# thecasterian/fluca

Hardware: AMD Instinct MI355X
Metric: pressure-Poisson Jacobi-PCG iterations/s, 512^3 cells per GPU (higher is better)
Workload: dtype f64

## Files before the change

fluca_amd/csrc/fl_cheb2.hip:

```cpp
#include <type_traits>

#include "fl_device.h"
#include "fl_handle.h"

namespace fl {

typedef double v2d_t __attribute__((ext_vector_type(2)));
template <int NT>
__device__ __forceinline__ double2 c2_ld2(const double *p)
{
  if (NT) {
    const v2d_t v = __builtin_nontemporal_load(reinterpret_cast<const v2d_t *>(p));
    return make_double2(v.x, v.y);
  }
  return *reinterpret_cast<const double2 *>(p);
}
template <int NT>
__device__ __forceinline__ void c2_st2(double *p, double2 v)
{
  if (NT) {
    v2d_t t;
    t.x = v.x;
    t.y = v.y;
    __builtin_nontemporal_store(t, reinterpret_cast<v2d_t *>(p));
  } else *reinterpret_cast<double2 *>(p) = v;
}

template <int NT>
__device__ __forceinline__ double2 c2_LD2(const double *base, unsigned byteoff) { return c2_ld2<NT>(reinterpret_cast<const double *>(reinterpret_cast<const char *>(base) + byteoff)); }
__device__ __forceinline__ double c2_LD1(const double *base, unsigned byteoff) { return *reinterpret_cast<const double *>(reinterpret_cast<const char *>(base) + byteoff); }
template <int NT>
__device__ __forceinline__ void c2_ST2(double *base, unsigned byteoff, double2 v) { c2_st2<NT>(reinterpret_cast<double *>(reinterpret_cast<char *>(base) + byteoff), v); }
__device__ __forceinline__ void c2_ST1(double *base, unsigned byteoff, double v) { *reinterpret_cast<double *>(reinterpret_cast<char *>(base) + byteoff) = v; }

__device__ __forceinline__ int c2_wrap(int gi, int n, int per, bool &in)
{
  if (gi < 0) {
    const int m = per & 3;
    in = m != 0;
    return m == 1 ? gi + n : (m == 2 ? gi : 0);
  }
  if (gi >= n) {
    const int m = (per >> 2) & 3;
    in = m != 0;
    return m == 1 ? gi - n : (m == 2 ? gi : n - 1);
  }
  in = true;
  return gi;
}

__device__ __forceinline__ int c2_xcd_remap(int b, int nblocks) { return (nblocks & 7) ? b : (b & 7) * (nblocks >> 3) + (b >> 3); }

template <int RY, int NW, bool JAC, int NT, bool MGD = false, int Z = 0>
__global__ void __launch_bounds__(64 * NW) k_cheb2(GridP g, int perx, int pery, int perz, const double *X0, const double *X1, double *X0w, double *X1w, const double *__restrict__ b, const double *D0, const double *D1, double *D0w,
                                                  double *D1w, const KspScal *__restrict__ s, double *__restrict__ partial, int stride, int zc, int tiles_x, int tiles, int remap, const double *__restrict__ zq = nullptr,
                                                  const double *__restrict__ za_dev = nullptr, double *__restrict__ bw = nullptr)
{
  constexpr bool ZR = Z != 0, ZS = Z == 2;
  static_assert(!(ZR && MGD), "the three-step sweep is the pre-smoother: no sums of the outer iteration");
  constexpr int TX = 128, TY = NW * RY, LX = TX + 4, NTH = 64 * NW;
  constexpr int NTL = NT >= 2, NTS = NT >= 1;
  __shared__ __attribute__((aligned(16))) double XJ[3][TY + 4][LX];
  __shared__ __attribute__((aligned(16))) double XN[3][TY + 2][LX];
  __shared__ double                              red[6 * NW], cB[2 * TY][5];
  if (s->reason != 0) return;

  const double *x  = s->cur ? X1 : X0;
  double       *xn = s->cur ? X0w : X1w;
  const double *d  = s->dcur ? D1 : D0;
  double       *dn = s->dcur ? D0w : D1w;
  double        rho0 = s->cheb_rho, c0 = s->cheb_c;
  double        rho1, c1;
  const double  cf = s->cheb_c;
  const double  za = ZS ? *za_dev : 0.;
  {
    double ck, ckm1;
    cheb_advance(s, s->ck, s->ckm1, ck, ckm1, rho1, c1);
    if (ZR) {
      rho0 = rho1;
      c0   = c1;
      double ck2, ckm2;
      cheb_advance(s, ck, ckm1, ck2, ckm2, rho1, c1);
    }
  }

  const int bb    = remap ? c2_xcd_remap(blockIdx.x, gridDim.x) : blockIdx.x;
  const int chunk = bb / tiles, tile = bb % tiles;
  const int i0 = (tile % tiles_x) * TX, j0 = (tile / tiles_x) * TY;
  const int k0 = chunk * zc, k1 = min(k0 + zc, g.nz);
  const int tid = threadIdx.x, lane = tid & 63;
  const int w   = __builtin_amdgcn_readfirstlane(tid >> 6);
  const int ie = min(TX, g.nx - i0), je = min(TY, g.ny - j0);
// ... 253 lines not shown
        const double2 below = *reinterpret_cast<const double2 *>(&XJ[bp][rlr][lc]);
        const double  west = XJ[bc][rlr][lc - 1], east = XJ[bc][rlr][lc + 2];
        const double  dyz = Ayc + z1c;
        const double  v0 = (xc0 + dyz) * cen.x + xl0 * west + xh0 * cen.y + Ayl * south.x + Ayh * north.x + z1l * below.x + z1h * C.hxR.x;
        const double  v1 = (xc1 + dyz) * cen.y + xl1 * cen.x + xh1 * east + Ayl * south.y + Ayh * north.y + z1l * below.y + z1h * C.hxR.y;
        const double2 bm = ZR ? zb1R : C.hbR, dm = ZR ? cen : C.hdR;
        const double  r0 = bm.x - v0, r1 = bm.y - v1;
        const double  z0 = JAC ? r0 / (xc0 + dyz) : r0, z1 = JAC ? r1 / (xc1 + dyz) : r1;
        const double  e0 = (rho0 != 0. ? rho0 * dm.x : 0.) + c0 * z0;
        const double  e1 = (rho0 != 0. ? rho0 * dm.y : 0.) + c0 * z1;
        hx1R.x = (rinn0 && pin1) ? cen.x + e0 : 0.;
        hx1R.y = (rinn1 && pin1) ? cen.y + e1 : 0.;
      }
      if (anyB) {
        const double cen = XJ[bc][HB.lr][HB.lc], dyz = cB[tbc][4] + z1c;
        const double v = dyz * cen + cB[tbc][0] * XJ[bc][HB.lr][HB.lc - 1] + cB[tbc][1] * XJ[bc][HB.lr][HB.lc + 1] + cB[tbc][2] * XJ[bc][HB.lr - 1][HB.lc] + cB[tbc][3] * XJ[bc][HB.lr + 1][HB.lc] + z1l * XJ[bp][HB.lr][HB.lc] + z1h * C.hxB;
        const double r = (ZR ? zb1B : C.hbB) - v, z = JAC ? r / dyz : r;
        const double e = (rho0 != 0. ? rho0 * (ZR ? cen : C.hdB) : 0.) + c0 * z;
        hx1B = (HB.in && pin1) ? cen + e : 0.;
      }
    }

    if constexpr (DO2) {
      const int     bc = (k2 + 3) % 3, bp = (k2 + 2) % 3;
      const int64_t p2 = (int64_t)k2 * g.sxy;
#pragma unroll
      for (int m = 0; m < RY; ++m) {
        const int     lr    = w * RY + m + 1;
        const double2 cen   = *reinterpret_cast<const double2 *>(&XN[bc][lr][lc]);
        const double2 south = *reinterpret_cast<const double2 *>(&XN[bc][lr - 1][lc]);
        const double2 north = *reinterpret_cast<const double2 *>(&XN[bc][lr + 1][lc]);
        const double2 below = *reinterpret_cast<const double2 *>(&XN[bp][lr][lc]);
        const double  west = XN[bc][lr][lc - 1], east = XN[bc][lr][lc + 2];
        const double  dyz = yc[m] + z2c;
        const double  v0 = (xc0 + dyz) * cen.x + xl0 * west + xh0 * cen.y + yl[m] * south.x + yh[m] * north.x + z2l * below.x + z2h * x1v[m].x;
        const double  v1 = (xc1 + dyz) * cen.y + xl1 * cen.x + xh1 * east + yl[m] * south.y + yh[m] * north.y + z2l * below.y + z2h * x1v[m].y;
        const double  r0 = sb2[m].x - v0, r1 = sb2[m].y - v1;
        const double  z0 = JAC ? r0 / (xc0 + dyz) : r0, z1 = JAC ? r1 / (xc1 + dyz) : r1;
        double2       e, xo;
        e.x  = rho1 * d1p[m].x + c1 * z0;
        e.y  = rho1 * d1p[m].y + c1 * z1;
        xo.x = cen.x + e.x;
        xo.y = cen.y + e.y;
        if (rin[m] && in0) {
          if (in1) {
            c2_ST2<NTS>(dn + rob[m] + p2, lo, e);
            c2_ST2<NTS>(xn + rob[m] + p2, lo, xo);
            if (MGD) {
              acc[0] += xo.x + xo.y;
              acc[1] += xo.x * xo.x + xo.y * xo.y;
              acc[2] += sb2[m].x * xo.x + sb2[m].y * xo.y;
              acc[3] += sb2[m].x + sb2[m].y;
              acc[4] += sb2[m].x * sb2[m].x + sb2[m].y * sb2[m].y;
            } else {
              acc[3] += z0 + z1;
              acc[4] += z0 * z0 + z1 * z1;
              acc[5] += r0 * r0 + r1 * r1;
            }
          } else {
            c2_ST1(dn + rob[m] + p2, lo, e.x);
            c2_ST1(xn + rob[m] + p2, lo, xo.x);
            if (MGD) {
              acc[0] += xo.x;
              acc[1] += xo.x * xo.x;
              acc[2] += sb2[m].x * xo.x;
              acc[3] += sb2[m].x;
              acc[4] += sb2[m].x * sb2[m].x;
            } else {
              acc[3] += z0;
              acc[4] += z0 * z0;
              acc[5] += r0 * r0;
            }
          }
        }
      }
    }

    {
      const int bj = (kk + 3) % 3, bn = (kc + 3) % 3;
#pragma unroll
      for (int m = 0; m < RY; ++m) {
        if (rin[m]) {
          if (in1) {
            *reinterpret_cast<double2 *>(&XJ[bj][w * RY + m + 2][lc]) = C.x[m];
            if constexpr (DO1) *reinterpret_cast<double2 *>(&XN[bn][w * RY + m + 1][lc]) = x1v[m];
          } else if (in0) {
            XJ[bj][w * RY + m + 2][lc] = C.x[m].x;
            if constexpr (DO1) XN[bn][w * RY + m + 1][lc] = x1v[m].x;
          }
        }
      }
      if (rok1) {
        *reinterpret_cast<double2 *>(&XJ[bj][rlr][lc]) = C.hxR;
        if constexpr (DO1)
          if (rowA) *reinterpret_cast<double2 *>(&XN[bn][rlr - 1][lc]) = hx1R;
      } else if (rok0) {
        XJ[bj][rlr][lc] = C.hxR.x;
        if constexpr (DO1)
          if (rowA) XN[bn][rlr - 1][lc] = hx1R.x;
      }
// ... 73 lines not shown
}

int fl_cheb2_agree(fl_poisson *h)
{
  if (h->cheb2_agreed[0] >= 0) return 0;
  const bool legal = fl_cheb2_usable(h);
  double     no[2] = {legal ? 0. : 1., (legal && h->ncell >= 32768) ? 0. : 1.};
  if (h->multi) {
    FL_CHK(fl_allreduce_sum(h, &no[0]));
    FL_CHK(fl_allreduce_sum(h, &no[1]));
  }
  h->cheb2_agreed[0] = no[0] == 0. ? 1 : 0;
  h->cheb2_agreed[1] = no[1] == 0. ? 1 : 0;
  return 0;
}

Cheb2Plan fl_cheb2_plan(const GridP &g)
{
  Cheb2Plan p;
  p.nw      = g.ny > 8 ? 8 : 4;
  p.tiles_x = (g.nx + 127) / 128;
  const int ty    = 2 * p.nw;
  const int tiles = p.tiles_x * ((g.ny + ty - 1) / ty);
  p.tiles         = tiles;
  int nchunk = z_chunk_count(tiles, g.nz, 256, 16);
  if (tiles * nchunk > 256 && tiles <= 256) nchunk = std::max(1, 256 / tiles);
  const ZChunks z = z_chunks(g.nz, nchunk);
  p.zc      = z.zc;
  p.nchunk  = z.nchunk;
  p.nblocks = tiles * p.nchunk;
  return p;
}

template <int NW, bool JAC, bool MGD = false, int Z = 0>
static void cheb2_t(fl_poisson *h, const Cheb2Plan &p, double *X0, double *X1, const double *B, double *D0, double *D1, const double *zq = nullptr, const double *za_dev = nullptr, double *bw = nullptr)
{
  int per[3];
  for (int d = 0; d < 3; ++d) {
    int m[2];
    for (int side = 0; side < 2; ++side) m[side] = (h->multi && h->nbr[2 * d + side] >= 0 && !h->wrap_local[d]) ? 2 : (h->ax[d].periodic ? 1 : 0);
    per[d] = m[0] | (m[1] << 2);
  }
  hipLaunchKernelGGL((k_cheb2<2, NW, JAC, 2, MGD, Z>), dim3(p.nblocks), dim3(64 * NW), 0, h->stream, h->g, per[0], per[1], per[2], X0, X1, X0, X1, B, D0, D1, D0, D1, h->scal, h->partial, h->partial_stride, p.zc, p.tiles_x, p.tiles, 1,
                     zq, za_dev, bw);
}

void fl_launch_cheb2_from_zero(fl_poisson *h, const Cheb2Plan &p, bool jac, double *X0, double *X1, const double *B, double *D0, double *D1, const double *subq, const double *suba_dev, double *Bw)
{
  if (subq) {
    if (p.nw == 8) {
      if (jac) cheb2_t<8, true, false, 2>(h, p, X0, X1, B, D0, D1, subq, suba_dev, Bw);
      else cheb2_t<8, false, false, 2>(h, p, X0, X1, B, D0, D1, subq, suba_dev, Bw);
    } else {
      if (jac) cheb2_t<4, true, false, 2>(h, p, X0, X1, B, D0, D1, subq, suba_dev, Bw);
      else cheb2_t<4, false, false, 2>(h, p, X0, X1, B, D0, D1, subq, suba_dev, Bw);
    }
    return;
  }
  if (p.nw == 8) {
    if (jac) cheb2_t<8, true, false, 1>(h, p, X0, X1, B, D0, D1);
    else cheb2_t<8, false, false, 1>(h, p, X0, X1, B, D0, D1);
  } else {
    if (jac) cheb2_t<4, true, false, 1>(h, p, X0, X1, B, D0, D1);
    else cheb2_t<4, false, false, 1>(h, p, X0, X1, B, D0, D1);
  }
}

void fl_launch_cheb2(fl_poisson *h, const Cheb2Plan &p, bool jac, double *X0, double *X1, const double *B, double *D0, double *D1, bool mgdots)
{
  if (mgdots) {
    if (p.nw == 8) cheb2_t<8, true, true>(h, p, X0, X1, B, D0, D1);
    else cheb2_t<4, true, true>(h, p, X0, X1, B, D0, D1);
    return;
  }
  if (p.nw == 8) {
    if (jac) cheb2_t<8, true>(h, p, X0, X1, B, D0, D1);
    else cheb2_t<8, false>(h, p, X0, X1, B, D0, D1);
  } else {
    if (jac) cheb2_t<4, true>(h, p, X0, X1, B, D0, D1);
    else cheb2_t<4, false>(h, p, X0, X1, B, D0, D1);
  }
}
```

fluca_amd/csrc/fl_handle.h:

```cpp
#pragma once
#include <algorithm>
#include <cmath>
#include <cstdlib>
#include <cstring>
#include <limits>
#include <list>
#include <string>

#include "fl_internal.h"
#include "fl_knobs.h"

typedef struct ncclComm *ncclComm_t;

namespace fl {

void launch_pad_copy(hipStream_t, const GridP &, const double *, double *);
void launch_unpad_copy(hipStream_t, const GridP &, const double *, double *, const double *);
void launch_project_all(hipStream_t, const GridP &, const double *p, double *const v[3], double *const V[3]);
bool project_six_usable(const GridP &, const double *p_unpadded, double *const v[3], double *const V[3]);
void launch_project_six(hipStream_t, const GridP &, const double *p, bool direct, int per, double *const v[3], double *const V[3]);
void launch_wrap(hipStream_t, const GridP &, double *, int axis, int nvec = 1, int64_t vstride = 0);
void launch_pack_faces_sr(hipStream_t, const GridP &, const double *r, const double *sb, const double *W, const KspScal *s, double *const bufs[6]);
void launch_face_ext(hipStream_t, const GridP &, double *v, double *buf, int axis, int side, int ea, int eb, int mode);
void launch_face_ext_deep(hipStream_t, const GridP &, double *v, double *buf, int axis, int side, int ea, int eb, int dp, int mode);
// ... 188 lines not shown
    *count_out = cnt;
  }
  ~ProfEvents()
  {
    for (hipEvent_t e : ev) (void)hipEventDestroy(e);
  }
};

inline int fl_plane_size(const fl_poisson *h, int d) { return d == 0 ? h->g.ny * h->g.nz : (d == 1 ? h->g.nx * h->g.nz : h->g.nx * h->g.ny); }
int  fl_dev_alloc(fl_poisson *h, void **p, size_t bytes, bool zero);
int  fl_ensure_vec(fl_poisson *h, double **v);
void fl_vmm_destroy(fl_poisson *h);
int  fl_ensure_partials(fl_poisson *h, int nblocks);
int  fl_ensure_hist(fl_poisson *h, int nhist);
int  fl_zero_vec(fl_poisson *h, double *v);
int  fl_halo_messages(const fl_poisson *h, bool self, fl_halo_msg plan[12]);
int  fl_fill_ghosts(fl_poisson *h, double *v);
int  fl_fill_ghosts_full(fl_poisson *h, double *v);
int  fl_fill_ghosts_deep(fl_poisson *h, double *v);
int  fl_fill_hifaces(fl_poisson *h, const double *const V[3]);
int  fl_exchange_r_begin(fl_poisson *h, double *r, const double *q);
int  fl_exchange_sr_begin(fl_poisson *h, const double *r, const double *sb, const double *W, double *rn);
int  fl_exchange_r_end(fl_poisson *h, double *r);
bool fl_any_ghost_exchange(const fl_poisson *h);
int fl_allreduce_max(fl_poisson *h, double *v);
int fl_allreduce_sum(fl_poisson *h, double *v);
int fl_poll_scal(fl_poisson *h);
int fl_apply_tiled(fl_poisson *h, const double *xpad, double *y, int unpadded_y);
int fl_residual(fl_poisson *h, const double *x, const double *b, double *r);
int fl_residual_padded(fl_poisson *h, double *xpad, const double *bpad, double *rpad);
bool fl_residual_restrict_fusable(const GridP &g);
int fl_residual_restrict_padded(fl_poisson *h, double *xpad, const double *bpad, const double *wx, const double *wy, const double *wz, fl_poisson *hc, double *cpad);
int fl_apply_padded_dot(fl_poisson *h, double *xpad, double *ypad, double *xy);
int fl_cheb_smooth_padded(fl_poisson *h, int nu, bool jac, bool guess_zero, bool *mgdots = nullptr, const double *subq = nullptr, const double *suba_dev = nullptr);
int fl_solve_cg(fl_poisson *h, const double *b, double *x, const fl_ksp_opts *o, fl_ksp_stats *st);
int fl_solve_bcgs(fl_poisson *h, const double *b, double *x, const fl_ksp_opts *o, fl_ksp_stats *st);
int fl_solve_cg_sr(fl_poisson *h, const double *b, double *x, const fl_ksp_opts *o, fl_ksp_stats *st);
int fl_ksp_begin(fl_poisson *h, const fl_ksp_opts *o);
int fl_bcgs_fin_step(fl_poisson *h, int mode, int nblocks, int nslot, int nhist);
int fl_ksp_finish(fl_poisson *h, const fl_ksp_opts *o, fl_ksp_stats *st);
int fl_cheb_begin(fl_poisson *h, const fl_ksp_opts *o, double emin, double emax);
int fl_cheb_fin_step(fl_poisson *h, int nblocks, int nhist);
int fl_solve_cheb(fl_poisson *h, const double *b, double *x, const fl_ksp_opts *o, fl_ksp_stats *st);
double fl_gershgorin_bound(const fl_poisson *h, bool jac);
struct Cheb2Plan {
  int nw, tiles_x, tiles, nchunk, zc, nblocks;
};
bool      fl_cheb2_usable(const fl_poisson *h);
int       fl_cheb2_agree(fl_poisson *h);
Cheb2Plan fl_cheb2_plan(const GridP &g);
void      fl_launch_cheb2(fl_poisson *h, const Cheb2Plan &p, bool jac, double *X0, double *X1, const double *B, double *D0, double *D1, bool mgdots = false);
namespace fl {
struct SchurVarT {
  const double *w0[3], *w1[3];
  const int    *c0[3];
};
}
bool      fl_schur_var_usable(const fl_poisson *h);
int       fl_schur_var_fill_ghosts(fl_poisson *h, double *p_pad);
int       fl_schur_var_apply_fused(fl_poisson *h, const fl::SchurVarT &t, const double *ainv, const double *p_pad, double *y);
struct SchurVarPlan {
  int     per_xcd, nseg, band, fixed_seg;
  int64_t items;
};
SchurVarPlan schur_var_plan(const fl::GridP &g);
struct TP {
  int ry, nchunk, zc, tiles_x, nblocks;
};
TP tile_plan(const fl::GridP &g);
void      fl_launch_cheb2_from_zero(fl_poisson *h, const Cheb2Plan &p, bool jac, double *X0, double *X1, const double *B, double *D0, double *D1, const double *subq, const double *suba_dev, double *Bw);
int  fl_solve_cg_mg(fl_poisson *h, const double *b, double *x, const fl_ksp_opts *o, fl_ksp_stats *st);
void fl_mg_destroy(fl_poisson *h);
void fl_mg_set_stream(fl_poisson *h);
```

fluca_amd/csrc/fl_knobs.h:

```cpp
#pragma once
#include <atomic>

#define FL_PUBLIC_KNOBS(X)                                                                                                                   \
  X(cheb_fuse, 1)                   \
  X(placement, 0)                           \
  X(cg_xbatch, 1)                                           \
  X(cg_xdepth, 8)                 \
  X(cheb_zero3, 1)                  \
  X(mg_prolong, 1)                                                             \
  X(mg_flexible, 1)                                                             \
  X(mg_coarse, 1)                                   \
  X(mg_post_smooth, 0)               \
  X(schur_var_fused, 1)      \
  X(overlap, 1)              \
  X(comm_loopback, 0)           \
  X(comm_trace, 0)                             \
  X(ghost_width, 0)                                       \
  X(placement_verbose, 0)                                                                        \
  X(placement_vmm, 1)                    \
  X(allreduce, 0)

namespace fl {

enum Knob : int {
#define X(n, d) K_##n,
  FL_PUBLIC_KNOBS(X)
#undef X
      K_COUNT
};

int         knob(Knob k);
void        knob_set(Knob k, int v);
int         knob_find(const char *name);
const char *knob_name(int k);

}
```

fluca_amd/csrc/fl_ksp.hip:

```cpp
#include <ctime>
#include "fl_handle.h"
#include "fl_device.h"
#include "fl_stencil.h"

namespace fl {

__device__ __forceinline__ double2 LD2(const double *base, unsigned byteoff) { return *reinterpret_cast<const double2 *>(reinterpret_cast<const char *>(base) + byteoff); }
__device__ __forceinline__ void    ST2(double *base, unsigned byteoff, double2 v) { *reinterpret_cast<double2 *>(reinterpret_cast<char *>(base) + byteoff) = v; }
__device__ __forceinline__ void    ST1(double *base, unsigned byteoff, double v) { *reinterpret_cast<double *>(reinterpret_cast<char *>(base) + byteoff) = v; }
__device__ __forceinline__ double uniform(double v)
{
  const int lo = __builtin_amdgcn_readfirstlane(__double2loint(v)), hi = __builtin_amdgcn_readfirstlane(__double2hiint(v));
  return __hiloint2double(hi, lo);
}


struct Tile {
  int  i, il, k0, k1, lane, w, j0w, i0;
  bool own0, own1;
};
template <int RY>
__device__ __forceinline__ Tile make_tile(const GridP &g, int nchunk, int zc, int tiles_x)
{
  Tile      t;
// ... 1045 lines not shown
  return !((g.nx & 1) || (g.ny & 1) || (g.nz & 1));
}

int fl_residual_restrict_padded(fl_poisson *h, double *xpad, const double *bpad, const double *wx, const double *wy, const double *wz, fl_poisson *hc, double *cpad)
{
  const GridP &g = h->g, &gc = hc->g;
  if (!fl_residual_restrict_fusable(g)) return 1;
  if (gc.nx * 2 != g.nx || gc.ny * 2 != g.ny || gc.nz * 2 != g.nz) return 1;
  const PlanA p = plan_cg_A(g, 0, 0);
  FL_CHK(fl_fill_ghosts(h, xpad));
  StAux ax;
  ax.csx  = gc.sx;
  ax.csxy = gc.sxy;
  ax.coff = gc.off0;
  if (p.nw == 8) bcgs_st_t<2, 8, 11>(h, p, false, xpad, bpad, wx, wy, cpad, const_cast<double *>(wz), ax);
  else bcgs_st_t<2, 4, 11>(h, p, false, xpad, bpad, wx, wy, cpad, const_cast<double *>(wz), ax);
  return 0;
}

int fl_apply_padded_dot(fl_poisson *h, double *xpad, double *ypad, double *xy)
{
  FL_CHK(fl_fill_ghosts(h, xpad));
  const PlanA pa = plan_cg_A(h->g, 0, 0);
  FL_CHK(fl_ensure_partials(h, pa.nblocks));
  launch_bcgs_st<7>(h, pa, false, xpad, nullptr, nullptr, nullptr, ypad, nullptr);
  launch_reduce(h->stream, h->partial, pa.nblocks, h->partial_stride, 4, h->sums);
  if (h->multi) FL_CHK(h->comm.allreduce(h->stream, h->sums, NSLOT));
  if (!xy) return 0;
  FL_HIP(hipMemcpyAsync(xy, h->sums + 2, sizeof(double), hipMemcpyDeviceToHost, h->stream));
  FL_HIP(hipStreamSynchronize(h->stream));
  return 0;
}

int fl_cheb_smooth_padded(fl_poisson *h, int nu, bool jac, bool guess_zero, bool *mgdots, const double *subq, const double *suba)
{
  if (subq && !(guess_zero && nu > 0)) return FL_ERR_ARG_WRONGSTATE;
  const bool want = mgdots && *mgdots;
  if (mgdots) *mgdots = false;
  for (double **v : {&h->r, &h->P0, &h->q, &h->xp}) FL_CHK(fl_ensure_vec(h, v));
  if (nu <= 0) {
    if (guess_zero) FL_CHK(fl_zero_vec(h, h->xp));
    return 0;
  }
  const TP tp = tile_plan(h->g);
  FL_CHK(fl_ensure_partials(h, std::max(tp.nblocks, 1024)));
  const int nhist = nu + 2;
  FL_CHK(fl_ensure_hist(h, nhist));
  hipStream_t  s = h->stream;
  fl_ksp_opts  o;
  fl_ksp_opts_default(&o);
  o.norm_type        = FL_NORM_NONE;
  o.maxit            = nu;
  o.remove_nullspace = 0;
  const double lam = fl_gershgorin_bound(h, jac), emin = 0.1 * lam, emax = 1.1 * lam;
  init_scal(h, &o);
  KspScal S0 = *h->scal_host;
  S0.scale     = 2. / (emax + emin);
  const double alpha = 1. - S0.scale * emin;
  S0.mu        = 1. / alpha;
  S0.omegaprod = 2. / alpha;
  S0.ckm1      = 1.;
  S0.ck        = S0.mu;
  S0.cheb_rho  = 0.;
  S0.cheb_c    = S0.scale;
  const int fuse_ok = cheb_fuse(h);
  if (fuse_ok < 0) return fuse_ok;
  const bool fuse = fuse_ok && nu - (guess_zero ? 1 : 0) >= 2;
  Cheb2Plan  cp{};
  if (fuse) {
    cp = fl_cheb2_plan(h->g);
    FL_CHK(fl_ensure_vec(h, &h->cd1));
// ... 48 lines not shown
          S.dcur ^= 1;
          S.it += 2;
          advance(S, ck, ckm1, S.ck, S.ckm1, rho2, c2);
          S.cheb_rho = rho2;
          S.cheb_c   = c2;
          j += 2;
        } else {
          double ck, ckm1, rho, c;
          S.cur ^= 1;
          S.it += 1;
          advance(S, S.ck, S.ckm1, ck, ckm1, rho, c);
          S.ck       = ck;
          S.ckm1     = ckm1;
          S.cheb_rho = rho;
          S.cheb_c   = c;
          j += 1;
        }
      }
      FL_HIP(hipMalloc((void **)&q.dev, sizeof(KspScal) * q.host.size()));
      h->smooth_seq.push_back(std::move(q));
      hit = &h->smooth_seq.back();
      FL_HIP(hipMemcpyAsync(hit->dev, hit->host.data(), sizeof(KspScal) * hit->host.size(), hipMemcpyHostToDevice, s));
    }
    seq = hit->dev;
  }
  struct ScalGuard {
    fl_poisson *h;
    KspScal    *keep;
    ~ScalGuard() { h->scal = keep; }
  } guard{h, h->scal};
  const bool deep = fuse && h->multi;
  bool       bghost = false;
  int        launch = 0;
  for (int j = 0; j < nu;) {
    h->scal = const_cast<KspScal *>(seq) + launch++;
    const int kind = kind_of(j);
    if (kind == 3) {
      double *Bw = nullptr;
      if (subq) {
        FL_CHK(fl_ensure_vec(h, &h->rb));
        Bw = h->rb;
      }
      fl_launch_cheb2_from_zero(h, cp, jac, X0, X1, B, D0, D1, subq, suba, Bw);
      if (subq) {
        std::swap(h->r, h->rb);
        B = h->r;
      }
      dcur ^= 1;
      j += 3;
    } else if (kind == 1) {
      const int64_t items = (int64_t)((h->g.nx + 127) / 128) * h->g.ny * h->g.nz;
      const int     nb    = (int)std::max<int64_t>(1, std::min<int64_t>((items + 3) / 4, 8192));
      if (subq) {
        if (jac) hipLaunchKernelGGL((k_cheb_first<true, true>), dim3(nb), dim3(256), 0, s, h->g, X0, X1, B, D0, D1, h->scal, subq, suba);
        else hipLaunchKernelGGL((k_cheb_first<false, true>), dim3(nb), dim3(256), 0, s, h->g, X0, X1, B, D0, D1, h->scal, subq, suba);
      } else if (jac) hipLaunchKernelGGL((k_cheb_first<true>), dim3(nb), dim3(256), 0, s, h->g, X0, X1, B, D0, D1, h->scal, (const double *)nullptr, (const double *)nullptr);
      else hipLaunchKernelGGL((k_cheb_first<false>), dim3(nb), dim3(256), 0, s, h->g, X0, X1, B, D0, D1, h->scal, (const double *)nullptr, (const double *)nullptr);
      j += 1;
    } else if (kind == 2) {
      const bool md = want && jac && j + 2 == nu && !h->multi;
      if (deep) {
        if (!bghost) FL_CHK(fl_fill_ghosts(h, B));
        bghost = true;
        FL_CHK(fl_fill_ghosts_deep(h, cur ? X1 : X0));
        FL_CHK(fl_fill_ghosts(h, dcur ? D1 : D0));
      }
      mark("ghosts filled, before fused", j);
      fl_launch_cheb2(h, cp, jac, X0, X1, B, D0, D1, md);
      mark("fused done", j);
      dcur ^= 1;
      if (md) {
        launch_reduce(s, h->partial, cp.nblocks, h->partial_stride, 5, h->sums);
        *mgdots = true;
      }
      j += 2;
    } else {
      if (ghosts) FL_CHK(fl_fill_ghosts(h, cur ? X1 : X0));
      mark("before single", j);
      (void)launch_cheb(h, tp, jac, X0, X1, B, D0, D1);
      mark("single done", j);
      j += 1;
    }
    cur ^= 1;
  }
  if (cur) std::swap(h->xp, h->P0);
  h->poisoned = true;
  return 0;
}


int fl_solve_cg(fl_poisson *h, const double *b, double *x, const fl_ksp_opts *o, fl_ksp_stats *st)
{
  if (o->variant != 0) return FL_ERR_SUP;
  const GridP &g   = h->g;
  const bool   jac = o->pc == FL_PC_JACOBI;
  for (double **v : {&h->r, &h->P0, &h->P1, &h->q, &h->xp}) FL_CHK(fl_ensure_vec(h, v));
  PlanA plan = plan_cg_A(g, 0, 0);
  plan.qb    = h->multi ? 1 : 0;
  const int   nsb  = stream_blocks(g);
  FL_CHK(fl_ensure_partials(h, std::max(nsb, plan.nblocks)));
  const int nhist = o->maxit + 1;
  FL_CHK(fl_ensure_hist(h, nhist));
  hipStream_t s = h->stream;

  const bool xbatch_env = knob(K_cg_xbatch) != 0;
  const bool xlazy  = xbatch_env;
// ... 304 lines not shown
```

fluca_amd/csrc/fl_mg.hip:

```cpp
#include <new>

#include "fl_handle.h"
#include "fl_device.h"

namespace fl {

struct Owned {
  int64_t npair_row, npairs;
};
__device__ __forceinline__ Owned owned_of(const GridP &g)
{
  Owned o;
  o.npair_row = (g.nx + 1) / 2;
  o.npairs    = o.npair_row * (int64_t)g.ny * g.nz;
  return o;
}
__device__ __forceinline__ int64_t pair_off(const GridP &g, const Owned &o, int64_t q, bool &two)
{
  const int     ip = (int)(q % o.npair_row);
  const int64_t row = q / o.npair_row;
  const int     j = (int)(row % g.ny), k = (int)(row / g.ny);
  two = 2 * ip + 1 < g.nx;
  return g.off0 + (int64_t)k * g.sxy + (int64_t)j * g.sx + 2 * ip;
}
// ... 191 lines not shown
  for (int64_t it = (int64_t)blockIdx.x * nw + w; it < nitem; it += (int64_t)gridDim.x * nw) {
    const int seg = (int)(it % nseg), row = (int)(it / nseg);
    const int j = row % g.ny, k = row / g.ny, i = seg * 128 + 2 * lane;
    if (i >= g.nx) continue;
    const bool    two = i + 1 < g.nx;
    const int64_t off = g.off0 + (int64_t)k * g.sxy + (int64_t)j * g.sx + i;
    if (OP == 0) {
      const double2 xv = ldp(x0, off, two), yv = ldp(y0, off, two);
      stp(y0, off, two, make_double2((xv.x - c) + b * yv.x, (xv.y - c) + b * yv.y));
    } else if (OP == 1) {
      const double2 pv = ldp(x0, off, two), qv = ldp(x1, off, two), xv = ldp(y0, off, two), rv = ldp(y1, off, two);
      stp(y0, off, two, make_double2(xv.x + a * pv.x, xv.y + a * pv.y));
      stp(y1, off, two, make_double2(rv.x - a * qv.x, rv.y - a * qv.y));
    } else if (OP == 3) {
      const double2 pv = ldp(x0, off, two), xv = ldp(y0, off, two);
      stp(y0, off, two, make_double2(xv.x + a * pv.x, xv.y + a * pv.y));
    } else if (OP == 4) {
      const double2 zv = ldp(x0, off, two), pv = ldp(y0, off, two), xv = ldp(y1, off, two);
      stp(y1, off, two, make_double2(xv.x + a * pv.x, xv.y + a * pv.y));
      stp(y0, off, two, make_double2((zv.x - c) + b * pv.x, (zv.y - c) + b * pv.y));
    } else if (OP == 5) {
      const double2 qv = ldp(x1, off, two), rv = ldp(y1, off, two);
      stp(y1, off, two, make_double2(rv.x - a * qv.x, rv.y - a * qv.y));
    } else {
      const double2 xv = ldp(x0, off, two);
      stp(y0, off, two, make_double2(xv.x - c, xv.y - c));
    }
  }
}

struct MgScal {
  double alpha, beta, m, rz, rz_old, pq, dp, N;
  int    ns, pnorm, bad_pq, pad_;
};
struct MgSlot {
  double dp, rz, pq;
  int    bad_pq, pad_;
};
template <int STEP, bool FIRST = false>
__global__ void k_mg_scal(MgScal *__restrict__ S, const double *__restrict__ sums, MgSlot *__restrict__ slot_dev)
{
  if (STEP == 0) {
    const double pq = sums[2];
    S->pq     = pq;
    S->bad_pq = !(pq > 0.);
    S->alpha  = pq > 0. ? S->rz / pq : 0.;
  } else if (STEP == 1) {
    const double d0 = sums[0], d1 = sums[1], d2 = sums[2], d3 = sums[3], d4 = sums[4], N = S->N;
    const double m  = S->ns ? d0 / N : 0.;
    const double zz = d1 - N * m * m;
    double       dp = S->pnorm ? sqrt(zz > 0. ? zz : 0.) : sqrt(d4);
    if (isnan(d1)) dp = d1;
    if (!FIRST) S->rz_old = S->rz;
    S->m  = m;
    S->dp = dp;
    S->rz = d2 - m * d3;
    slot_dev->dp     = dp;
    slot_dev->rz     = S->rz;
    slot_dev->pq     = S->pq;
    slot_dev->bad_pq = FIRST ? 0 : S->bad_pq;
  } else if (STEP == 2) {
    S->beta = -S->alpha * (sums[2] - S->m * sums[3]) / S->rz_old;
  } else {
    S->beta = S->rz / S->rz_old;
  }
}

__global__ void k_mg_scal_set(MgScal *dst, MgScal v) { *dst = v; }

constexpr int MG_COARSE_MAX = 4096, MG_COARSE_CPT = MG_COARSE_MAX / 256;
__global__ void __launch_bounds__(256) k_mg_coarse_cg(GridP g, int perbits, int ns, double rtol, double atol, double dtol, int maxit, const double *__restrict__ b, double *__restrict__ x)
{
  constexpr int CPT = MG_COARSE_CPT;
  __shared__ double P[MG_COARSE_MAX];
  __shared__ double red[4 * 4], bc[4];
  const int tid = threadIdx.x, n = g.nx * g.ny * g.nz;
  double    xr[CPT], rr[CPT], di[CPT];
  int       cell_i[CPT], cell_j[CPT], cell_k[CPT];
  auto sum4 = [&](double (&v)[4]) {
    block_sum<4>(v, red);
    if (tid == 0)
#pragma unroll
      for (int a = 0; a < 4; ++a) bc[a] = v[a];
    __syncthreads();
#pragma unroll
    for (int a = 0; a < 4; ++a) v[a] = bc[a];
    __syncthreads();
  };
#pragma unroll
  for (int m = 0; m < CPT; ++m) {
    const int c = tid + 256 * m, cc = min(c, n - 1);
    const int i = cc % g.nx, t = cc / g.nx, j = t % g.ny, k = t / g.ny;
    cell_i[m] = i;
    cell_j[m] = j;
    cell_k[m] = k;
// ... 233 lines not shown
        };
        for (int64_t il = 0; il < hf->dec.len[d]; ++il) {
          const int64_t i = hf->dec.lo[d] + il, I = i / 2, In = (i % 2) ? I + 1 : I - 1;
          if (!hf->ax[d].periodic && (In < 0 || In >= nc)) continue;
          const double xc = 0.5 * (hf->ax[d].xf[(size_t)i] + hf->ax[d].xf[(size_t)i + 1]);
          pn[(size_t)il] = (i % 2) ? 1 : -1;
          pw[(size_t)il] = (xc - Xc(I)) / (Xc(In) - Xc(I));
        }
      }
      FL_HIP(hipMalloc((void **)&mg->lv[l].pn[d], sizeof(int) * std::max<size_t>(pn.size(), 1)));
      FL_HIP(hipMalloc((void **)&mg->lv[l].pw[d], sizeof(double) * std::max<size_t>(pw.size(), 1)));
      FL_HIP(hipMemcpy(mg->lv[l].pn[d], pn.data(), sizeof(int) * pn.size(), hipMemcpyHostToDevice));
      FL_HIP(hipMemcpy(mg->lv[l].pw[d], pw.data(), sizeof(double) * pw.size(), hipMemcpyHostToDevice));
    }
  }
  for (size_t l = 0; l < mg->lv.size(); ++l) {
    MgLevel    &L = mg->lv[l];
    fl_poisson *hl = L.h;
    for (double **v : {&hl->r, &hl->P0, &hl->q, &hl->xp}) FL_CHK(fl_ensure_vec(hl, v));
    if (l + 1 == mg->lv.size()) {
      FL_CHK(alloc_cells(hl, &L.x));
      FL_CHK(alloc_cells(hl, &L.b));
    }
    FL_CHK(fl_ensure_partials(hl, MG_BLOCKS));
  }
  for (double **v : {&h->w0, &h->w1, &h->w2}) FL_CHK(fl_ensure_vec(h, v));
  FL_HIP(hipMalloc((void **)&mg->scal, sizeof(MgScal)));
  FL_HIP(hipMalloc((void **)&mg->slot_dev, 2 * sizeof(MgSlot)));
  FL_HIP(hipHostMalloc((void **)&mg->slot_host, 2 * sizeof(MgSlot)));
  for (hipEvent_t &e : mg->ev_slot) FL_HIP(hipEventCreateWithFlags(&e, hipEventDisableTiming));
  return 0;
}

int vcycle(fl_mg *mg, size_t l, const fl_ksp_opts *o, bool *sums = nullptr, const double *subq = nullptr)
{
  const bool want = sums && *sums;
  if (sums) *sums = false;
  MgLevel    &L = mg->lv[l];
  fl_poisson *h = L.h;
  if (l + 1 == mg->lv.size()) {
    fl_ksp_stats st;
    fl_ksp_opts  so;
    fl_ksp_opts_default(&so);
    so.remove_nullspace = o->remove_nullspace;
    so.type  = FL_KSP_CG;
    so.pc    = FL_PC_JACOBI;
    so.rtol  = 1e-2;
    so.maxit = 200;
    if (subq) hipLaunchKernelGGL(k_mg_pwd<5>, dim3(nblk_pairs(h->g)), dim3(256), 0, h->stream, h->g, (const MgScal *)mg->scal, (const double *)nullptr, subq, (double *)nullptr, h->r);
    if (!h->multi && h->ncell <= MG_COARSE_MAX && fl_mg_coarse_mode() != 0) {
      const int per = (h->ax[0].periodic ? 1 : 0) | (h->ax[1].periodic ? 2 : 0) | (h->ax[2].periodic ? 4 : 0);
      hipLaunchKernelGGL(k_mg_coarse_cg, dim3(1), dim3(256), 0, h->stream, h->g, per, so.remove_nullspace, so.rtol, so.atol, so.dtol, so.maxit, (const double *)h->r, h->xp);
      return 0;
    }
    launch_unpad_copy(h->stream, h->g, h->r, L.b, nullptr);
    if (l == 0) {
      FL_CHK(fl_ensure_vec(h, &h->cd1));
      FL_HIP(hipMemcpyAsync(h->cd1, h->r, sizeof(double) * h->padlen, hipMemcpyDeviceToDevice, h->stream));
    }
    FL_CHK(fl_poisson_solve(h, L.b, L.x, &so, &st));
    if (l == 0) FL_HIP(hipMemcpyAsync(h->r, h->cd1, sizeof(double) * h->padlen, hipMemcpyDeviceToDevice, h->stream));
    launch_pad_copy(h->stream, h->g, L.x, h->xp);
    return 0;
  }
  const int nu = o->mg_smooth_its > 0 ? o->mg_smooth_its : 3;
  MgLevel  &C  = mg->lv[l + 1];
  FL_CHK(fl_cheb_smooth_padded(h, nu, true, true, nullptr, subq, subq ? &mg->scal->alpha : nullptr));
  int fused = 1;
  if (L.r[0] == 2 && L.r[1] == 2 && L.r[2] == 2) {
    fused = fl_residual_restrict_padded(h, h->xp, h->r, L.w[0], L.w[1], L.w[2], C.h, C.h->r);
    if (fused < 0) return fused;
  }
  if (fused != 0) {
    FL_CHK(fl_residual_padded(h, h->xp, h->r, h->q));
    hipLaunchKernelGGL(k_mg_restrict, dim3(nblk(C.h->ncell)), dim3(256), 0, h->stream, C.h->g, h->g, L.r[0], L.r[1], L.r[2], L.w[0], L.w[1], L.w[2], h->q, C.h->r);
  }
  FL_CHK(vcycle(mg, l + 1, o));
  if (fl_mg_prolong_mode() == 1) {
    FL_CHK(fl_fill_ghosts_full(C.h, C.h->xp));
    MgLin t;
    for (int d = 0; d < 3; ++d) {
      t.pn[d] = L.pn[d];
      t.pw[d] = L.pw[d];
    }
    if (L.r[0] == 2 && L.r[1] == 2 && L.r[2] == 2) {
      const int  kc = 4;
      const GridP &gcs = C.h->g;
      hipLaunchKernelGGL(k_mg_prolong_lin_cc, dim3((gcs.nx + 61) / 62, (gcs.ny + 3) / 4, (gcs.nz + kc - 1) / kc), dim3(256), 0, h->stream, h->g, gcs, t, (const double *)C.h->xp, h->xp, kc);
    } else {
      const int  zc = 8;
      const dim3 grid((h->g.nx + 127) / 128, (h->g.ny + 3) / 4, (h->g.nz + zc - 1) / zc);
      hipLaunchKernelGGL(k_mg_prolong_lin_tile, grid, dim3(256), 0, h->stream, h->g, C.h->g, L.r[0], L.r[1], L.r[2], t, (const double *)C.h->xp, h->xp, zc);
    }
  } else hipLaunchKernelGGL(k_mg_prolong_add, dim3(nblk_pairs(h->g)), dim3(256), 0, h->stream, h->g, C.h->g, L.r[0], L.r[1], L.r[2], C.h->xp, h->xp);
  bool got = want;
  const int nu_post = knob(K_mg_post_smooth) > 0 ? knob(K_mg_post_smooth) : nu;
  FL_CHK(fl_cheb_smooth_padded(h, nu_post, true, false, &got));
  if (sums) *sums = got;
  return 0;
}

}

void fl_mg_destroy(fl_poisson *h)
{
  fl_mg *mg = h->mg;
  if (!mg) return;
  for (size_t l = 0; l < mg->lv.size(); ++l) {
    MgLevel &L = mg->lv[l];
    for (double *p : {L.x, L.b, L.w[0], L.w[1], L.w[2], L.pw[0], L.pw[1], L.pw[2]})
      if (p) (void)hipFree(p);
    for (int *p : L.pn)
      if (p) (void)hipFree(p);
    if (l > 0 && L.h) fl_poisson_destroy(L.h);
  }
  if (mg->scal) (void)hipFree(mg->scal);
  if (mg->slot_dev) (void)hipFree(mg->slot_dev);
  if (mg->slot_host) (void)hipHostFree(mg->slot_host);
  for (hipEvent_t e : mg->ev_slot)
    if (e) (void)hipEventDestroy(e);
  delete mg;
  h->mg = nullptr;
}

void fl_mg_set_stream(fl_poisson *h)
{
  if (!h->mg) return;
  for (size_t l = 1; l < h->mg->lv.size(); ++l) (void)fl_poisson_set_stream(h->mg->lv[l].h, (void *)h->stream);
}

// ... 17 lines not shown
  struct Events {
    hipEvent_t a = nullptr, b = nullptr;
    ~Events()
    {
      if (a) (void)hipEventDestroy(a);
      if (b) (void)hipEventDestroy(b);
    }
  } ev;
  FL_HIP(hipEventCreate(&ev.a));
  FL_HIP(hipEventCreate(&ev.b));
  hipEvent_t e0 = ev.a, e1 = ev.b;
  FL_HIP(hipEventRecord(e0, s));
  double *X = h->w0, *P = h->w1, *Q = h->w2;
  double  d[5], rz = 0., dp = 0., pq = 0.;
  int     bad_pq = 0;
  std::vector<double> hist;
  MgScal *S = mg->scal;
  {
    MgScal init;
    std::memset(&init, 0, sizeof(init));
    init.N      = N;
    init.ns     = ns ? 1 : 0;
    init.pnorm  = pnorm ? 1 : 0;
    init.rz_old = 1.;
    hipLaunchKernelGGL(k_mg_scal_set, dim3(1), dim3(1), 0, s, S, init);
  }
  auto dots_dev = [&](const double *z, const double *r) -> int {
    hipLaunchKernelGGL(k_mg_dots, dim3(nb), dim3(256), 0, s, g, z, r, h->partial, h->partial_stride);
    launch_reduce(s, h->partial, nb, h->partial_stride, 5, h->sums);
    if (h->multi) FL_CHK(h->comm.allreduce(s, h->sums, NSLOT));
    return 0;
  };
  const double *subq = nullptr;
  auto cycle_and_sums = [&](int it, bool first) -> int {
    bool got = true;
    FL_CHK(vcycle(mg, 0, o, &got, subq));
    if (!got) FL_CHK(dots_dev(h->xp, h->r));
    const int a = it & 1;
    if (first) hipLaunchKernelGGL((k_mg_scal<1, true>), dim3(1), dim3(1), 0, s, S, (const double *)h->sums, mg->slot_dev + a);
    else hipLaunchKernelGGL((k_mg_scal<1, false>), dim3(1), dim3(1), 0, s, S, (const double *)h->sums, mg->slot_dev + a);
    FL_HIP(hipMemcpyAsync(mg->slot_host + a, mg->slot_dev + a, sizeof(MgSlot), hipMemcpyDeviceToHost, s));
    FL_HIP(hipEventRecord(mg->ev_slot[a], s));
    return 0;
  };
  auto look = [&](int it) -> int {
    const int a = it & 1;
    FL_HIP(hipEventSynchronize(mg->ev_slot[a]));
    const MgSlot &L = mg->slot_host[a];
    dp     = L.dp;
    rz     = L.rz;
    pq     = L.pq;
    bad_pq = L.bad_pq;
    return 0;
  };
  launch_pad_copy(s, g, b, h->r);
  FL_CHK(fl_zero_vec(h, X));
  FL_CHK(cycle_and_sums(0, true));
  hipLaunchKernelGGL(k_mg_pwd<2>, dim3(nb), dim3(256), 0, s, g, (const MgScal *)S, (const double *)h->xp, (const double *)nullptr, P, (double *)nullptr);
  FL_CHK(look(0));
  const double rnorm0 = dp, ttol = std::max(o->rtol * dp, o->atol);
  hist.push_back(dp);
  int  it = 0, reason = 0;
  auto converged = [&](double v) {
    if (std::isnan(v) || std::isinf(v)) return (int)FL_DIVERGED_NANORINF;
    if (v <= ttol) return v < o->atol ? (int)FL_CONVERGED_ATOL : (int)FL_CONVERGED_RTOL;
    if (v >= o->dtol * rnorm0) return (int)FL_DIVERGED_DTOL;
    return 0;
  };
  reason = converged(dp);
  if (!reason && o->maxit <= 0) reason = FL_DIVERGED_ITS;
  const bool flexible = fl_mg_flexible_mode() != 0;
  while (!reason) {
    FL_CHK(fl_apply_padded_dot(h, P, Q, nullptr));
    hipLaunchKernelGGL((k_mg_scal<0>), dim3(1), dim3(1), 0, s, S, (const double *)h->sums, (MgSlot *)nullptr);
    subq = Q;
    FL_CHK(cycle_and_sums(it + 1, false));
    subq = nullptr;
    if (flexible) {
      FL_CHK(dots_dev(h->xp, Q));
      hipLaunchKernelGGL((k_mg_scal<2>), dim3(1), dim3(1), 0, s, S, (const double *)h->sums, (MgSlot *)nullptr);
    } else hipLaunchKernelGGL((k_mg_scal<3>), dim3(1), dim3(1), 0, s, S, (const double *)h->sums, (MgSlot *)nullptr);
    hipLaunchKernelGGL(k_mg_pwd<4>, dim3(nb), dim3(256), 0, s, g, (const MgScal *)S, (const double *)h->xp, (const double *)nullptr, P, X);
    FL_CHK(look(it + 1));
    if (bad_pq) {
      reason = std::isnan(pq) ? FL_DIVERGED_NANORINF : FL_DIVERGED_INDEFINITE_MAT;
      break;
    }
    ++it;
    hist.push_back(dp);
    reason = converged(dp);
    if (!reason && it >= o->maxit) reason = FL_DIVERGED_ITS;
    if (!reason && !(rz > 0.)) reason = std::isnan(rz) ? FL_DIVERGED_NANORINF : FL_DIVERGED_INDEFINITE_PC;
  }
  double *shift = nullptr;
  if (ns) {
    FL_CHK(dots(h, X, X, d));
    const double mx = d[0] / N;
    FL_HIP(hipMemcpyAsync(h->sums, &mx, sizeof(double), hipMemcpyHostToDevice, s));
    FL_HIP(hipStreamSynchronize(s));
    shift = h->sums;
  }
  launch_unpad_copy(s, g, X, x, shift);
  FL_HIP(hipEventRecord(e1, s));
  FL_HIP(hipStreamSynchronize(s));
  float ms = 0.f;
  FL_HIP(hipEventElapsedTime(&ms, e0, e1));
  st->iters   = it;
  st->reason  = reason;
  if (reason == FL_DIVERGED_NANORINF || reason == FL_DIVERGED_DTOL || !std::isfinite(dp)) {
    for (MgLevel &L : mg->lv) L.h->poisoned = true;
  } else {
// ... 12 lines not shown
```

Baseline: 725.6.

## Skip dead direction stores in final Chebyshev sweeps and fuse flexible-CG q-dot into smoother

Adds an ND template flag so the last fused Chebyshev sweep skips writing the direction vector, which no later step reads. Adds a QD flag that accumulates q·x in the final post-smoother's reduction, using the sum of P saved from the apply step. Flexible-CG can then compute beta without a separate dots kernel and reduction pass over the fine grid. Both are gated by a new mg_lean knob, on by default, which costs extra template instantiations and one extra q load per cell in the fused sweep.

```diff
diff --git a/fluca_amd/csrc/fl_cheb2.hip b/fluca_amd/csrc/fl_cheb2.hip
--- a/fluca_amd/csrc/fl_cheb2.hip
+++ b/fluca_amd/csrc/fl_cheb2.hip
@@ -51,13 +51,14 @@
 
 __device__ __forceinline__ int c2_xcd_remap(int b, int nblocks) { return (nblocks & 7) ? b : (b & 7) * (nblocks >> 3) + (b >> 3); }
 
-template <int RY, int NW, bool JAC, int NT, bool MGD = false, int Z = 0>
+template <int RY, int NW, bool JAC, int NT, bool MGD = false, int Z = 0, bool ND = false, bool QD = false>
 __global__ void __launch_bounds__(64 * NW) k_cheb2(GridP g, int perx, int pery, int perz, const double *X0, const double *X1, double *X0w, double *X1w, const double *__restrict__ b, const double *D0, const double *D1, double *D0w,
                                                   double *D1w, const KspScal *__restrict__ s, double *__restrict__ partial, int stride, int zc, int tiles_x, int tiles, int remap, const double *__restrict__ zq = nullptr,
                                                   const double *__restrict__ za_dev = nullptr, double *__restrict__ bw = nullptr)
 {
   constexpr bool ZR = Z != 0, ZS = Z == 2;
   static_assert(!(ZR && MGD), "the three-step sweep is the pre-smoother: no sums of the outer iteration");
+  static_assert(!QD || MGD, "q.x'' is one of the outer iteration's sums");
   constexpr int TX = 128, TY = NW * RY, LX = TX + 4, NTH = 64 * NW;
   constexpr int NTL = NT >= 2, NTS = NT >= 1;
   __shared__ __attribute__((aligned(16))) double XJ[3][TY + 4][LX];
@@ -377,6 +378,8 @@
         const double2 north = *reinterpret_cast<const double2 *>(&XN[bc][lr + 1][lc]);
         const double2 below = *reinterpret_cast<const double2 *>(&XN[bp][lr][lc]);
         const double  west = XN[bc][lr][lc - 1], east = XN[bc][lr][lc + 2];
+        double2 qv = make_double2(0., 0.);
+        if (QD) qv = c2_LD2<NTL>(zq + rob[m] + p2, lo);
         const double  dyz = yc[m] + z2c;
         const double  v0 = (xc0 + dyz) * cen.x + xl0 * west + xh0 * cen.y + yl[m] * south.x + yh[m] * north.x + z2l * below.x + z2h * x1v[m].x;
         const double  v1 = (xc1 + dyz) * cen.y + xl1 * cen.x + xh1 * east + yl[m] * south.y + yh[m] * north.y + z2l * below.y + z2h * x1v[m].y;
@@ -389,7 +392,7 @@
         xo.y = cen.y + e.y;
         if (rin[m] && in0) {
           if (in1) {
-            c2_ST2<NTS>(dn + rob[m] + p2, lo, e);
+            if (!ND) c2_ST2<NTS>(dn + rob[m] + p2, lo, e);
             c2_ST2<NTS>(xn + rob[m] + p2, lo, xo);
             if (MGD) {
               acc[0] += xo.x + xo.y;
@@ -397,13 +400,14 @@
               acc[2] += sb2[m].x * xo.x + sb2[m].y * xo.y;
               acc[3] += sb2[m].x + sb2[m].y;
               acc[4] += sb2[m].x * sb2[m].x + sb2[m].y * sb2[m].y;
+              if (QD) acc[5] += qv.x * xo.x + qv.y * xo.y;
             } else {
               acc[3] += z0 + z1;
               acc[4] += z0 * z0 + z1 * z1;
               acc[5] += r0 * r0 + r1 * r1;
             }
           } else {
-            c2_ST1(dn + rob[m] + p2, lo, e.x);
+            if (!ND) c2_ST1(dn + rob[m] + p2, lo, e.x);
             c2_ST1(xn + rob[m] + p2, lo, xo.x);
             if (MGD) {
               acc[0] += xo.x;
@@ -411,6 +415,7 @@
               acc[2] += sb2[m].x * xo.x;
               acc[3] += sb2[m].x;
               acc[4] += sb2[m].x * sb2[m].x;
+              if (QD) acc[5] += qv.x * xo.x;
             } else {
               acc[3] += z0;
               acc[4] += z0 * z0;
@@ -550,7 +555,7 @@
   return p;
 }
 
-template <int NW, bool JAC, bool MGD = false, int Z = 0>
+template <int NW, bool JAC, bool MGD = false, int Z = 0, bool ND = false, bool QD = false>
 static void cheb2_t(fl_poisson *h, const Cheb2Plan &p, double *X0, double *X1, const double *B, double *D0, double *D1, const double *zq = nullptr, const double *za_dev = nullptr, double *bw = nullptr)
 {
   int per[3];
@@ -559,43 +564,54 @@
     for (int side = 0; side < 2; ++side) m[side] = (h->multi && h->nbr[2 * d + side] >= 0 && !h->wrap_local[d]) ? 2 : (h->ax[d].periodic ? 1 : 0);
     per[d] = m[0] | (m[1] << 2);
   }
-  hipLaunchKernelGGL((k_cheb2<2, NW, JAC, 2, MGD, Z>), dim3(p.nblocks), dim3(64 * NW), 0, h->stream, h->g, per[0], per[1], per[2], X0, X1, X0, X1, B, D0, D1, D0, D1, h->scal, h->partial, h->partial_stride, p.zc, p.tiles_x, p.tiles, 1,
-                     zq, za_dev, bw);
-}
-
-void fl_launch_cheb2_from_zero(fl_poisson *h, const Cheb2Plan &p, bool jac, double *X0, double *X1, const double *B, double *D0, double *D1, const double *subq, const double *suba_dev, double *Bw)
+  hipLaunchKernelGGL((k_cheb2<2, NW, JAC, 2, MGD, Z, ND, QD>), dim3(p.nblocks), dim3(64 * NW), 0, h->stream, h->g, per[0], per[1], per[2], X0, X1, X0, X1, B, D0, D1, D0, D1, h->scal, h->partial, h->partial_stride, p.zc, p.tiles_x,
+                     p.tiles, 1, zq, za_dev, bw);
+}
+template <int NW, bool JAC, bool MGD = false, int Z = 0>
+static void cheb2_nd(fl_poisson *h, const Cheb2Plan &p, bool nod, double *X0, double *X1, const double *B, double *D0, double *D1, const double *zq = nullptr, const double *za_dev = nullptr, double *bw = nullptr)
+{
+  if constexpr (JAC) {
+    if (nod) return cheb2_t<NW, JAC, MGD, Z, true>(h, p, X0, X1, B, D0, D1, zq, za_dev, bw);
+  }
+  cheb2_t<NW, JAC, MGD, Z>(h, p, X0, X1, B, D0, D1, zq, za_dev, bw);
+}
+
+void fl_launch_cheb2_from_zero(fl_poisson *h, const Cheb2Plan &p, bool jac, double *X0, double *X1, const double *B, double *D0, double *D1, const double *subq, const double *suba_dev, double *Bw, bool nod)
 {
   if (subq) {
     if (p.nw == 8) {
-      if (jac) cheb2_t<8, true, false, 2>(h, p, X0, X1, B, D0, D1, subq, suba_dev, Bw);
-      else cheb2_t<8, false, false, 2>(h, p, X0, X1, B, D0, D1, subq, suba_dev, Bw);
+      if (jac) cheb2_nd<8, true, false, 2>(h, p, nod, X0, X1, B, D0, D1, subq, suba_dev, Bw);
+      else cheb2_nd<8, false, false, 2>(h, p, nod, X0, X1, B, D0, D1, subq, suba_dev, Bw);
     } else {
-      if (jac) cheb2_t<4, true, false, 2>(h, p, X0, X1, B, D0, D1, subq, suba_dev, Bw);
-      else cheb2_t<4, false, false, 2>(h, p, X0, X1, B, D0, D1, subq, suba_dev, Bw);
+      if (jac) cheb2_nd<4, true, false, 2>(h, p, nod, X0, X1, B, D0, D1, subq, suba_dev, Bw);
+      else cheb2_nd<4, false, false, 2>(h, p, nod, X0, X1, B, D0, D1, subq, suba_dev, Bw);
     }
     return;
   }
   if (p.nw == 8) {
-    if (jac) cheb2_t<8, true, false, 1>(h, p, X0, X1, B, D0, D1);
-    else cheb2_t<8, false, false, 1>(h, p, X0, X1, B, D0, D1);
+    if (jac) cheb2_nd<8, true, false, 1>(h, p, nod, X0, X1, B, D0, D1);
+    else cheb2_nd<8, false, false, 1>(h, p, nod, X0, X1, B, D0, D1);
   } else {
-    if (jac) cheb2_t<4, true, false, 1>(h, p, X0, X1, B, D0, D1);
-    else cheb2_t<4, false, false, 1>(h, p, X0, X1, B, D0, D1);
-  }
-}
-
-void fl_launch_cheb2(fl_poisson *h, const Cheb2Plan &p, bool jac, double *X0, double *X1, const double *B, double *D0, double *D1, bool mgdots)
+    if (jac) cheb2_nd<4, true, false, 1>(h, p, nod, X0, X1, B, D0, D1);
+    else cheb2_nd<4, false, false, 1>(h, p, nod, X0, X1, B, D0, D1);
+  }
+}
+
+void fl_launch_cheb2(fl_poisson *h, const Cheb2Plan &p, bool jac, double *X0, double *X1, const double *B, double *D0, double *D1, bool mgdots, bool nod, const double *dotq)
 {
   if (mgdots) {
-    if (p.nw == 8) cheb2_t<8, true, true>(h, p, X0, X1, B, D0, D1);
-    else cheb2_t<4, true, true>(h, p, X0, X1, B, D0, D1);
+    if (dotq) {
+      if (p.nw == 8) nod ? cheb2_t<8, true, true, 0, true, true>(h, p, X0, X1, B, D0, D1, dotq) : cheb2_t<8, true, true, 0, false, true>(h, p, X0, X1, B, D0, D1, dotq);
+      else nod ? cheb2_t<4, true, true, 0, true, true>(h, p, X0, X1, B, D0, D1, dotq) : cheb2_t<4, true, true, 0, false, true>(h, p, X0, X1, B, D0, D1, dotq);
+    } else if (p.nw == 8) cheb2_nd<8, true, true>(h, p, nod, X0, X1, B, D0, D1);
+    else cheb2_nd<4, true, true>(h, p, nod, X0, X1, B, D0, D1);
     return;
   }
   if (p.nw == 8) {
-    if (jac) cheb2_t<8, true>(h, p, X0, X1, B, D0, D1);
-    else cheb2_t<8, false>(h, p, X0, X1, B, D0, D1);
+    if (jac) cheb2_nd<8, true>(h, p, nod, X0, X1, B, D0, D1);
+    else cheb2_nd<8, false>(h, p, nod, X0, X1, B, D0, D1);
   } else {
-    if (jac) cheb2_t<4, true>(h, p, X0, X1, B, D0, D1);
-    else cheb2_t<4, false>(h, p, X0, X1, B, D0, D1);
-  }
-}
+    if (jac) cheb2_nd<4, true>(h, p, nod, X0, X1, B, D0, D1);
+    else cheb2_nd<4, false>(h, p, nod, X0, X1, B, D0, D1);
+  }
+}
diff --git a/fluca_amd/csrc/fl_handle.h b/fluca_amd/csrc/fl_handle.h
--- a/fluca_amd/csrc/fl_handle.h
+++ b/fluca_amd/csrc/fl_handle.h
@@ -244,7 +244,8 @@
 bool fl_residual_restrict_fusable(const GridP &g);
 int fl_residual_restrict_padded(fl_poisson *h, double *xpad, const double *bpad, const double *wx, const double *wy, const double *wz, fl_poisson *hc, double *cpad);
 int fl_apply_padded_dot(fl_poisson *h, double *xpad, double *ypad, double *xy);
-int fl_cheb_smooth_padded(fl_poisson *h, int nu, bool jac, bool guess_zero, bool *mgdots = nullptr, const double *subq = nullptr, const double *suba_dev = nullptr);
+int fl_cheb_smooth_padded(fl_poisson *h, int nu, bool jac, bool guess_zero, bool *mgdots = nullptr, const double *subq = nullptr, const double *suba_dev = nullptr,
+                          const double *dotq = nullptr, bool *gotq = nullptr);
 int fl_solve_cg(fl_poisson *h, const double *b, double *x, const fl_ksp_opts *o, fl_ksp_stats *st);
 int fl_solve_bcgs(fl_poisson *h, const double *b, double *x, const fl_ksp_opts *o, fl_ksp_stats *st);
 int fl_solve_cg_sr(fl_poisson *h, const double *b, double *x, const fl_ksp_opts *o, fl_ksp_stats *st);
@@ -261,7 +262,8 @@
 bool      fl_cheb2_usable(const fl_poisson *h);
 int       fl_cheb2_agree(fl_poisson *h);
 Cheb2Plan fl_cheb2_plan(const GridP &g);
-void      fl_launch_cheb2(fl_poisson *h, const Cheb2Plan &p, bool jac, double *X0, double *X1, const double *B, double *D0, double *D1, bool mgdots = false);
+void      fl_launch_cheb2(fl_poisson *h, const Cheb2Plan &p, bool jac, double *X0, double *X1, const double *B, double *D0, double *D1, bool mgdots = false, bool nod = false,
+                          const double *dotq = nullptr);
 namespace fl {
 struct SchurVarT {
   const double *w0[3], *w1[3];
@@ -280,7 +282,7 @@
   int ry, nchunk, zc, tiles_x, nblocks;
 };
 TP tile_plan(const fl::GridP &g);
-void      fl_launch_cheb2_from_zero(fl_poisson *h, const Cheb2Plan &p, bool jac, double *X0, double *X1, const double *B, double *D0, double *D1, const double *subq, const double *suba_dev, double *Bw);
+void      fl_launch_cheb2_from_zero(fl_poisson *h, const Cheb2Plan &p, bool jac, double *X0, double *X1, const double *B, double *D0, double *D1, const double *subq, const double *suba_dev, double *Bw, bool nod = false);
 int  fl_solve_cg_mg(fl_poisson *h, const double *b, double *x, const fl_ksp_opts *o, fl_ksp_stats *st);
 void fl_mg_destroy(fl_poisson *h);
 void fl_mg_set_stream(fl_poisson *h);
diff --git a/fluca_amd/csrc/fl_knobs.h b/fluca_amd/csrc/fl_knobs.h
--- a/fluca_amd/csrc/fl_knobs.h
+++ b/fluca_amd/csrc/fl_knobs.h
@@ -10,6 +10,7 @@
   X(mg_prolong, 1)                                                             \
   X(mg_flexible, 1)                                                             \
   X(mg_coarse, 1)                                   \
+  X(mg_lean, 3)            \
   X(mg_post_smooth, 0)               \
   X(schur_var_fused, 1)      \
   X(overlap, 1)              \
diff --git a/fluca_amd/csrc/fl_ksp.hip b/fluca_amd/csrc/fl_ksp.hip
--- a/fluca_amd/csrc/fl_ksp.hip
+++ b/fluca_amd/csrc/fl_ksp.hip
@@ -1101,11 +1101,13 @@
   return 0;
 }
 
-int fl_cheb_smooth_padded(fl_poisson *h, int nu, bool jac, bool guess_zero, bool *mgdots, const double *subq, const double *suba)
+int fl_cheb_smooth_padded(fl_poisson *h, int nu, bool jac, bool guess_zero, bool *mgdots, const double *subq, const double *suba, const double *dotq, bool *gotq)
 {
   if (subq && !(guess_zero && nu > 0)) return FL_ERR_ARG_WRONGSTATE;
   const bool want = mgdots && *mgdots;
   if (mgdots) *mgdots = false;
+  if (gotq) *gotq = false;
+  if (!gotq) dotq = nullptr;
   for (double **v : {&h->r, &h->P0, &h->q, &h->xp}) FL_CHK(fl_ensure_vec(h, v));
   if (nu <= 0) {
     if (guess_zero) FL_CHK(fl_zero_vec(h, h->xp));
@@ -1220,6 +1222,7 @@
   const bool deep = fuse && h->multi;
   bool       bghost = false;
   int        launch = 0;
+  const bool lean_d = (knob(K_mg_lean) & 1) != 0;
   for (int j = 0; j < nu;) {
     h->scal = const_cast<KspScal *>(seq) + launch++;
     const int kind = kind_of(j);
@@ -1229,7 +1232,7 @@
         FL_CHK(fl_ensure_vec(h, &h->rb));
         Bw = h->rb;
       }
-      fl_launch_cheb2_from_zero(h, cp, jac, X0, X1, B, D0, D1, subq, suba, Bw);
+      fl_launch_cheb2_from_zero(h, cp, jac, X0, X1, B, D0, D1, subq, suba, Bw, lean_d && j + 3 == nu);
       if (subq) {
         std::swap(h->r, h->rb);
         B = h->r;
@@ -1254,12 +1257,13 @@
         FL_CHK(fl_fill_ghosts(h, dcur ? D1 : D0));
       }
       mark("ghosts filled, before fused", j);
-      fl_launch_cheb2(h, cp, jac, X0, X1, B, D0, D1, md);
+      fl_launch_cheb2(h, cp, jac, X0, X1, B, D0, D1, md, lean_d && j + 2 == nu, md ? dotq : nullptr);
       mark("fused done", j);
       dcur ^= 1;
       if (md) {
-        launch_reduce(s, h->partial, cp.nblocks, h->partial_stride, 5, h->sums);
+        launch_reduce(s, h->partial, cp.nblocks, h->partial_stride, dotq ? 6 : 5, h->sums);
         *mgdots = true;
+        if (dotq) *gotq = true;
       }
       j += 2;
     } else {
diff --git a/fluca_amd/csrc/fl_mg.hip b/fluca_amd/csrc/fl_mg.hip
--- a/fluca_amd/csrc/fl_mg.hip
+++ b/fluca_amd/csrc/fl_mg.hip
@@ -247,6 +247,7 @@
 struct MgScal {
   double alpha, beta, m, rz, rz_old, pq, dp, N;
   int    ns, pnorm, bad_pq, pad_;
+  double sq;
 };
 struct MgSlot {
   double dp, rz, pq;
@@ -257,6 +258,7 @@
 {
   if (STEP == 0) {
     const double pq = sums[2];
+    S->sq     = sums[0];
     S->pq     = pq;
     S->bad_pq = !(pq > 0.);
     S->alpha  = pq > 0. ? S->rz / pq : 0.;
@@ -276,6 +278,8 @@
     slot_dev->bad_pq = FIRST ? 0 : S->bad_pq;
   } else if (STEP == 2) {
     S->beta = -S->alpha * (sums[2] - S->m * sums[3]) / S->rz_old;
+  } else if (STEP == 4) {
+    S->beta = -S->alpha * (sums[5] - S->m * S->sq) / S->rz_old;
   } else {
     S->beta = S->rz / S->rz_old;
   }
@@ -575,10 +579,11 @@
   return 0;
 }
 
-int vcycle(fl_mg *mg, size_t l, const fl_ksp_opts *o, bool *sums = nullptr, const double *subq = nullptr)
+int vcycle(fl_mg *mg, size_t l, const fl_ksp_opts *o, bool *sums = nullptr, const double *subq = nullptr, bool *qdot = nullptr)
 {
   const bool want = sums && *sums;
   if (sums) *sums = false;
+  if (qdot) *qdot = false;
   MgLevel    &L = mg->lv[l];
   fl_poisson *h = L.h;
   if (l + 1 == mg->lv.size()) {
@@ -638,7 +643,8 @@
   } else hipLaunchKernelGGL(k_mg_prolong_add, dim3(nblk_pairs(h->g)), dim3(256), 0, h->stream, h->g, C.h->g, L.r[0], L.r[1], L.r[2], C.h->xp, h->xp);
   bool got = want;
   const int nu_post = knob(K_mg_post_smooth) > 0 ? knob(K_mg_post_smooth) : nu;
-  FL_CHK(fl_cheb_smooth_padded(h, nu_post, true, false, &got));
+  const bool askq = qdot && subq && want && !h->multi && (knob(K_mg_lean) & 2) != 0 && fl_mg_flexible_mode() != 0;
+  FL_CHK(fl_cheb_smooth_padded(h, nu_post, true, false, &got, nullptr, nullptr, askq ? subq : nullptr, askq ? qdot : nullptr));
   if (sums) *sums = got;
   return 0;
 }
@@ -722,9 +728,10 @@
     return 0;
   };
   const double *subq = nullptr;
+  bool gotq = false;
   auto cycle_and_sums = [&](int it, bool first) -> int {
     bool got = true;
-    FL_CHK(vcycle(mg, 0, o, &got, subq));
+    FL_CHK(vcycle(mg, 0, o, &got, subq, &gotq));
     if (!got) FL_CHK(dots_dev(h->xp, h->r));
     const int a = it & 1;
     if (first) hipLaunchKernelGGL((k_mg_scal<1, true>), dim3(1), dim3(1), 0, s, S, (const double *)h->sums, mg->slot_dev + a);
@@ -766,7 +773,9 @@
     subq = Q;
     FL_CHK(cycle_and_sums(it + 1, false));
     subq = nullptr;
-    if (flexible) {
+    if (flexible && gotq) {
+      hipLaunchKernelGGL((k_mg_scal<4>), dim3(1), dim3(1), 0, s, S, (const double *)h->sums, (MgSlot *)nullptr);
+    } else if (flexible) {
       FL_CHK(dots_dev(h->xp, Q));
       hipLaunchKernelGGL((k_mg_scal<2>), dim3(1), dim3(1), 0, s, S, (const double *)h->sums, (MgSlot *)nullptr);
     } else hipLaunchKernelGGL((k_mg_scal<3>), dim3(1), dim3(1), 0, s, S, (const double *)h->sums, (MgSlot *)nullptr);
```

Result: no change. 720.0 (-0.8%).
